# NAIST-Archlab/vsim

Hardware: AMD Instinct MI355X
Metric: decode tokens/sec GPT-J-6B Q4_0 @1 GPU; achieved HBM GB/s vs peak (higher is better)
Workload: dtype f32 (Q4_0 x Q4_0 operands); 1 GPU; gpt-j-6B Q4_0 decode, 874 timed tokens after a 5-token prompt + 5 warm-up tokens, batch 1; mode=exact, n_ctx=980, parallelism=single, graph=True

## Files before the change

vsim_amd/csrc/common.hpp:

```cpp
#pragma once

#include <hip/hip_runtime.h>
#include <stdint.h>

#include <map>
#include <string>

#include "../../include/vsim_hip.h"

namespace vsim {

constexpr int QK = 32;
constexpr int QBYTES = 20;

constexpr int T32 = 32;

typedef float f32x4 __attribute__((ext_vector_type(4)));
typedef unsigned int u32x4 __attribute__((ext_vector_type(4)));

struct W4 {
  const uint8_t *qs;
  const float *d;
  int rows, k, tiles;
  __host__ __device__ int nb() const { return k / QK; }
  __host__ __device__ size_t off(int r, int b) const {
    return ((size_t)(r / T32) * nb() + b) * T32 + (r & (T32 - 1));
  }
};

inline size_t w4_bytes(int rows, int k) { return (size_t)((rows + T32 - 1) / T32) * T32 * (k / QK) * QBYTES; }

inline W4 w4_view(const void *base, int rows, int k) {
  W4 v;
  v.rows = rows;
  v.k = k;
  v.tiles = (rows + T32 - 1) / T32;
  const size_t nblk = (size_t)v.tiles * T32 * (k / QK);
  v.qs = (const uint8_t *)base;
  v.d = (const float *)((const uint8_t *)base + nblk * 16);
  return v;
}

enum { EPI_STORE = 0, EPI_GELU_Q = 1 };
struct GemvJob {
  W4 w;
  const float *xd;
  const uint8_t *xqs;
  const float *xdd;
  const float *bias;
  float *y;
  int epi;
  const uint16_t *gelu_tab;
  uint8_t *oq_qs;
  float *oq_d;
  float *oxd;
};
struct GemvBatch {
  GemvJob j[4];
  int nj;
};

struct LnQuantJob {
  const float *x;
  const float *w, *b;
  uint8_t *qs;
  float *d;
  float *xd;
  const float *ja, *jab, *jf, *jfb;
  float *jout;
  unsigned *ep;
};

struct TailLn {
  const float *x;
  const float *ab, *fb;
  float *jout;
  const float *w1, *b1;
  uint8_t *q1;
  float *d1, *xd1;
  const float *w2, *b2;
  uint8_t *q2;
  float *d2, *xd2;
  unsigned long long *og, *jg;
  uint4 *rec;
  const unsigned *ep;
  unsigned *stats;
  int il;
};
constexpr int LNT_MAX_TILES = 256;

struct AttnJob {
  const float *q, *k, *v;
  float *kc, *vc;
  const int *npast;
  const double2 *cs;
  const uint16_t *etab;
  int d, H, n_rot, style;
  int n_ctx;
  int nsplit;
  int kqv_nth;
  float scale;
  const float *alibi;
  uint8_t *oq_qs;
  float *oq_d, *oxd;
  float *out;
};

constexpr int ATT_VTF = 8192;
__host__ __device__ constexpr int attn_lds_floats(int d, int n_ctx) {
  return ((2 * d + n_ctx + 3) & ~3) + 2 * ATT_VTF;
}

int launch_ln_quant(const LnQuantJob &j0, const LnQuantJob *j1, int n, hipStream_t s);
int launch_residual_join(const float *x, const float *a, const float *ab, const float *f, const float *fb, float *out,
                         int n, hipStream_t s);
int launch_gemv_epi(const GemvBatch &B, int mode, hipStream_t s);
int launch_attn_decode(const AttnJob &A, int n_ctx, hipStream_t s);
struct AttnRows {
  float *const *kc, *const *vc;
  size_t loff;
  const int *npast;
};
int launch_attn_decode_batch(const AttnJob &A, const AttnRows &R, int B, int n_ctx, hipStream_t s);
int launch_gemv_chain_batch(const GemvBatch &B, hipStream_t s);
bool gemv_chain_solo(const GemvBatch &B);

__device__ __forceinline__ float bits_f(uint32_t w) { return __uint_as_float(w); }
__device__ __forceinline__ uint32_t f_bits(float f) { return __float_as_uint(f); }

__device__ __forceinline__ float h2f(uint16_t h) {
  const uint32_t w = (uint32_t)h << 16;
  const uint32_t sign = w & 0x80000000u;
  const uint32_t two_w = w + w;
  const float normalized = bits_f((two_w >> 4) + (0xE0u << 23)) * 0x1.0p-112f;
  const float denormalized = bits_f((two_w >> 17) | (126u << 23)) - 0.5f;
  return bits_f(sign | (two_w < (1u << 27) ? f_bits(denormalized) : f_bits(normalized)));
}

__device__ __forceinline__ uint16_t f2h(float f) {
  float base = (fabsf(f) * 0x1.0p+112f) * 0x1.0p-110f;
  const uint32_t w = f_bits(f);
  const uint32_t shl1_w = w + w;
  const uint32_t sign = w & 0x80000000u;
  uint32_t bias = shl1_w & 0xFF000000u;
  if (bias < 0x71000000u) bias = 0x71000000u;
  base = bits_f((bias >> 1) + 0x07800000u) + base;
  const uint32_t bits = f_bits(base);
  const uint32_t exp_bits = (bits >> 13) & 0x00007C00u;
  const uint32_t mantissa_bits = bits & 0x00000FFFu;
  const uint32_t nonsign = exp_bits + mantissa_bits;
  return (uint16_t)((sign >> 16) | (shl1_w > 0xFF000000u ? 0x7E00u : nonsign));
}

// ... 188 lines not shown
```

vsim_amd/csrc/gemv_chain.hip:

```cpp
#include <cstdlib>
#include <cstring>

#ifdef VSIM_NB_STAMPS
namespace vsim {
__device__ unsigned long long g_nb_stamps[2048][32];
}
#define ATT_STAMP(i) \
  if (threadIdx.x == 0) g_nb_stamps[1536 + blockIdx.x][4 + (i)] = __builtin_amdgcn_s_memrealtime()
#endif
#include "attn.hpp"
#include "kern.hpp"
#include "../../include/vsim_hip.h"

namespace vsim {

typedef const __attribute__((address_space(4))) float sfloat;
typedef const __attribute__((address_space(1))) u32x4 gu32x4;
typedef const __attribute__((address_space(1))) float gfloat;

__device__ __forceinline__ void producer_barrier() { asm volatile("s_barrier" ::: "memory"); }


constexpr int waitcnt_vm(int n) { return 0x0F70 | (n & 15) | ((n >> 4) << 14); }
constexpr int c2_waves(int npw, bool fill) {
// ... 726 lines not shown
        break;
      }
    }
  }
  __syncthreads();
  NBS(if (threadIdx.x == 0) tl[1] = __builtin_amdgcn_s_memrealtime();)
  if (T.lnon)
    chain32_nb_body<C2Tail, true, true, 2>(T.o, b, L.n, T.err, &T.ln);
  else
    chain32_nb_body<C2Tail, true, true>(T.o, b, L.n, T.err);
  NBS(if (threadIdx.x == 0) tl[2] = __builtin_amdgcn_s_memrealtime();)
}

bool tail_ln_ok(int E) {
  int dev = 0, cus = 0;
  if (hipGetDevice(&dev) != hipSuccess || hipDeviceGetAttribute(&cus, hipDeviceAttributeMultiprocessorCount, dev) != hipSuccess)
    return false;
  return E % T32 == 0 && E / T32 <= LNT_MAX_TILES && E / T32 < cus;
}

int launch_layer_tail(const GemvBatch &f, const GemvBatch &o, const AttnJob &a, const TailSync &sy, int n_ctx,
                      hipStream_t s, const TailLn *ln) {
  const int S = a.nsplit > 1 ? a.nsplit : 1;
  if (a.d % 32 != 0 || a.d > 256 || a.n_ctx != n_ctx || a.d % S != 0 || (a.d / S) % QK != 0 ||
      (size_t)attn_lds_floats(a.d, n_ctx) * sizeof(float) > sizeof(NbLds<C2Tail>)) {
    set_error("layer tail: attention shape (head dim, n_ctx) outside the fused kernel's range");
    return VSIM_EINVAL;
  }
  if (f.nj > 1 || o.nj > 1) {
    set_error("layer tail: fc_out and the out-projection are one job each");
    return VSIM_EINVAL;
  }
  TailJob T{};
  T.f = f;
  T.o = o;
  T.a = a;
  T.sy = sy;
  if (!sy.hflag || !sy.ep || sy.il < 0 || sy.il > 254 || a.H * S > TAIL_MAX_HEADS) {
    set_error("layer tail: the heads' flags need a flag buffer, the step epoch, a layer below 255, at most 128 heads");
    return VSIM_EINVAL;
  }
  T.err = spin_error_counter();
  T.nf = 0;
  if (ln) {
    const int E = o.nj == 1 ? o.j[0].w.rows : 0;
    if (f.nj != 1 || o.nj != 1 || f.j[0].w.rows != E || a.d * a.H != E || !tail_ln_ok(E) || ln->il < 0 ||
        ln->il > 254 || !ln->x || !ln->jout || !ln->w1 || !ln->b1 || !ln->q1 || !ln->d1 || !ln->xd1 || !ln->og ||
        !ln->jg || !ln->rec || !ln->ep || (ln->w2 && (!ln->b2 || !ln->q2 || !ln->d2 || !ln->xd2))) {
      set_error("layer tail: the in-tail LayerNorm needs fc_out and the out-projection over E rows, E/32 below the CU count");
      return VSIM_EINVAL;
    }
    T.lnon = 1;
    T.ln = *ln;
  }
  for (int i = 0; i < f.nj; ++i) T.nf += f.j[i].w.tiles;
  int no = 0;
  for (int i = 0; i < o.nj; ++i) no += o.j[i].w.tiles;
  const dim3 grid(T.nf + a.H * S + no), blk(C2Tail::THREADS);
  constexpr size_t pad = sizeof(NbLds<C2Tail>) > 80 * 1024 ? 0 : 81 * 1024 - sizeof(NbLds<C2Tail>);
  hipLaunchKernelGGL(k_layer_tail, grid, blk, pad, s, T);
  VSIM_HIP(hipGetLastError());
  return VSIM_OK;
}

template <int CB, int CONS = 1>
struct SoloShape {
  static constexpr int CP = CB * 16, LD = CP + 4;
  static constexpr int PRODUCERS = CB * CONS;
  static constexpr int WAVES = PRODUCERS + (PRODUCERS + 2) / 3;
  static constexpr int ROWS = 64 * CONS;
  static constexpr int WIN = 12;
  static_assert(CP / 4 % WIN == 0, "the read window must tile the chunk");
  static_assert(WAVES <= 16, "workgroup size");
  static_assert((WAVES + 3) / 4 >= CONS, "consumer waves on one SIMD");
};
constexpr int C5_RING = 3;

template <int CB, int PF, int CONS>
__device__ __forceinline__ void solo_body(const GemvBatch &B, int g, float (*P)[SoloShape<CB, CONS>::ROWS * SoloShape<CB, CONS>::LD]) {
  using S = SoloShape<CB, CONS>;
  constexpr int TPG = 2 * CONS;
  const int wave = __builtin_amdgcn_readfirstlane(threadIdx.x >> 6);
  const int lane = threadIdx.x & 63;
  int ji = 0;
  while (ji < B.nj) {
    const int ng = (B.j[ji].w.tiles + TPG - 1) / TPG;
    if (g < ng) break;
    g -= ng;
    ++ji;
  }
  if (ji >= B.nj) return;
  ji = __builtin_amdgcn_readfirstlane(ji);
  g = __builtin_amdgcn_readfirstlane(g);
  const int tiles = B.j[ji].w.tiles, nb = B.j[ji].w.k / QK, nch = (nb + CB - 1) / CB;
  const int nit = (nch + 2 + PF) / (PF + 1) * (PF + 1);
  NBS(if (lane == 0 && gridDim.x < 512 && wave < 32) g_nb_stamps[512 + blockIdx.x][wave] =
          (unsigned long long)__builtin_amdgcn_s_getreg(0xF804) | (unsigned long long)__builtin_amdgcn_s_getreg(0xF814) << 32;)

  if ((wave & 3) == 0 && (wave >> 2) >= CONS) {
    for (int k = 0; k < nit; ++k) __syncthreads();
    return;
  }
  if ((wave & 3) != 0) {
    const int pi = wave - 1 - (wave >> 2);
    const int o = pi % CB, c = pi / CB;
    const int h = lane >> 5, r = lane & 31;
    const int tile = TPG * g + 2 * c + h;
    const bool tile_ok = tile < tiles;
    const int tl = tile_ok ? tile : tiles - 1;
    const uint8_t *qs = B.j[ji].w.qs + ((size_t)tl * nb * T32 + r) * 16;
    const float *dd = B.j[ji].w.d + (size_t)tl * nb * T32 + r;
    const float *xg = B.j[ji].xd;
    auto ld = [&](int c, u32x4 &qv, float &dv) {
      const int b = min(c * CB + o, nb - 1);
      qv = __builtin_nontemporal_load((gu32x4 *)(qs + (size_t)b * (T32 * 16)));
      dv = __builtin_nontemporal_load((gfloat *)(dd + (size_t)b * T32));
    };
    auto ldx = [&](int c, f32x2 *xv) {
      const int b = min(c * CB + o, nb - 1);
      const sfloat *xp = (const sfloat *)(xg + (size_t)b * QK);
#pragma unroll
      for (int i = 0; i < 16; ++i) {
        xv[i].x = xp[2 * i];
        xv[i].y = xp[2 * i + 1];
      }
    };
    int ps = 0;
    NBS(unsigned long long st_fw = 0, st_comp = 0, st_bar = 0, pa = 0, pb = 0, pc = 0, pd = 0;
        auto cyc = []() { return __builtin_amdgcn_s_memtime(); };)
    auto step = [&](int k, const f32x2 *xc, f32x2 *xn, const u32x4 &qc, float dqc, u32x4 &qn, float &dqn) {
      ld(k + PF, qn, dqn);
      NBS(const unsigned long long c0 = cyc();)
      __builtin_amdgcn_s_waitcnt(0xC07F);
      NBS(if (pa) { st_fw += pb - pa; st_comp += pc - pb; st_bar += pd - pc; }
          pa = c0; pb = cyc();)
      __builtin_amdgcn_sched_barrier(0);
      ldx(k + 1, xn);
      __builtin_amdgcn_sched_barrier(0);
      {
        const float dv = tile_ok && k * CB + o < nb ? dqc : 0.0f;
        const float dl = 512.0f * dv, ml = -8.0f * dv;
        float dh, mh;
        asm("v_mov_b32 %0, %1" : "=v"(dh) : "v"(dl));
        asm("v_mov_b32 %0, %1" : "=v"(mh) : "v"(ml));
        const f32x2 d2 = {dl, dh}, m2 = {ml, mh};
        float *dst = &P[ps][(64 * c + lane) * S::LD + o * 16];
#pragma unroll
        for (int wv = 0; wv < 4; ++wv) {
          float p4[4];
          pair_terms4_x(qc[wv], d2, m2, xc + 4 * wv, p4);
          *(float4 *)(dst + 4 * wv) = make_float4(p4[0], p4[1], p4[2], p4[3]);
        }
      }
      ps = ps == C5_RING - 1 ? 0 : ps + 1;
      __builtin_amdgcn_sched_barrier(0);
      NBS(pc = cyc();)
      producer_barrier();
      NBS(pd = cyc();)
    };
    u32x4 q[PF + 1];
    float e[PF + 1];
#pragma unroll
    for (int c = 0; c < PF; ++c) ld(c, q[c], e[c]);
    f32x2 xa[16], xb[16];
    ldx(0, xa);
#pragma unroll
    for (int i = 0; i < 16; ++i) asm volatile("" ::"s"(xa[i].x), "s"(xa[i].y));
    static_assert((PF + 1) % 2 == 0, "two factor sets alternate");
    for (int k = 0; k < nit; k += PF + 1) {
#pragma unroll
      for (int u = 0; u < PF + 1; u += 2) {
        step(k + u, xa, xb, q[u], e[u], q[(u + PF) % (PF + 1)], e[(u + PF) % (PF + 1)]);
        step(k + u + 1, xb, xa, q[u + 1], e[u + 1], q[u % (PF + 1)], e[u % (PF + 1)]);
      }
    }
    NBS(if (lane == 0 && gridDim.x < 512 && pi < 6) {
      unsigned long long *st = g_nb_stamps[512 + blockIdx.x] + 12 + 3 * pi;
      st[0] = st_fw;
      st[1] = st_comp;
      st[2] = st_bar;
    })
    return;
  }

  float acc = 0.0f;
  float4 win[S::WIN];
  NBS(unsigned long long sc_bar = 0;
      auto ccyc = []() { return __builtin_amdgcn_s_memtime(); };)
  const int crow = 64 * wave / 4 + lane;
  auto src = [&](int c) { return &P[c % C5_RING][crow * S::LD]; };
  __builtin_amdgcn_s_setprio(3);
  NBS(const unsigned long long c_m0 = __builtin_amdgcn_s_memtime(), c_r0 = __builtin_amdgcn_s_memrealtime();)
  for (int k = 0; k < nit; ++k) {
    const int c = k - 2;
    if (c == -1 && nch > 0) {
      const float *p0 = src(0);
#pragma unroll
      for (int j = 0; j < S::WIN; ++j) win[j] = *(const float4 *)(p0 + 4 * j);
    } else if (c >= 0 && c < nch) {
      const float *pc = src(c), *pn = src(c + 1);
#pragma unroll
      for (int j0 = 0; j0 < S::CP / 4; j0 += 6) {
#pragma unroll
        for (int j = j0; j < j0 + 6; ++j) {
          const float4 v = win[j % S::WIN];
          acc = acc + v.x;
          acc = acc + v.y;
          acc = acc + v.z;
          acc = acc + v.w;
        }
#pragma unroll
        for (int j = j0; j < j0 + 6; ++j) {
          const int jn = j + S::WIN;
          win[j % S::WIN] = jn < S::CP / 4 ? *(const float4 *)(pc + 4 * jn) : *(const float4 *)(pn + 4 * (jn - S::CP / 4));
        }
        __builtin_amdgcn_sched_group_barrier(0x002, 24, 0);
        __builtin_amdgcn_sched_group_barrier(0x100, 6, 0);
      }
    }
    NBS(const unsigned long long b0 = ccyc();)
    __syncthreads();
    NBS(sc_bar += ccyc() - b0;)
  }
  NBS(if (lane == 0 && wave == 0 && gridDim.x < 512) {
    g_nb_stamps[512 + blockIdx.x][30] = sc_bar;
    g_nb_stamps[512 + blockIdx.x][31] = nit;
  })
  NBS(if (lane == 0 && wave == 0 && gridDim.x < 512) {
    unsigned long long *st = g_nb_stamps[512 + blockIdx.x];
    st[8] = c_m0;
    st[9] = __builtin_amdgcn_s_memtime();
    st[10] = c_r0;
    st[11] = __builtin_amdgcn_s_memrealtime();
  })

  const int row = g * S::ROWS + crow;
  const int rows = B.j[ji].w.rows;
  const float *bias = B.j[ji].bias;
  float *y = B.j[ji].y;
  if (B.j[ji].epi == EPI_GELU_Q) {
    const bool ok = row < rows;
    float gv = 0.0f;
    if (ok) {
      gv = h2f(B.j[ji].gelu_tab[f2h(acc + bias[row])]);
      if (y) y[row] = gv;
    }
    const int blk = row / QK;
    quantize_half(gv, lane, ok, B.j[ji].oq_qs + (size_t)blk * 16, B.j[ji].oq_d + blk,
                  B.j[ji].oxd + (size_t)blk * QK);
  } else if (row < rows) {
    y[row] = bias ? acc + bias[row] : acc;
  }
  __builtin_amdgcn_s_setprio(0);
}

template <int CB, int PF, int CONS>
__global__ void __launch_bounds__((64 * SoloShape<CB, CONS>::WAVES), 1) k_gemv_solo(GemvBatch B) {
  __shared__ __attribute__((aligned(16))) float P[C5_RING][SoloShape<CB, CONS>::ROWS * SoloShape<CB, CONS>::LD];
  solo_body<CB, PF, CONS>(B, blockIdx.x, P);
}

static int solo_groups(const GemvBatch &B, int cons = 1) {
  int g = 0;
  for (int i = 0; i < B.nj; ++i) g += (B.j[i].w.tiles + 2 * cons - 1) / (2 * cons);
  return g;
}

constexpr int SOLO_CB = 6, SOLO_PF = 3, SOLO_MIN_GROUPS = 192;

bool gemv_chain_solo(const GemvBatch &B) { return solo_groups(B) >= SOLO_MIN_GROUPS; }

int launch_gemv_chain_batch(const GemvBatch &B, hipStream_t s) {
  int tiles = 0;
  for (int i = 0; i < B.nj; ++i) {
    if (B.j[i].w.k % QK != 0 || B.j[i].w.k <= 0) {
      set_error("gemv: K must be a positive multiple of 32");
      return VSIM_EINVAL;
    }
    if (!B.j[i].xd) { set_error("gemv: exact mode needs the activation factors xd"); return VSIM_EINVAL; }
    tiles += B.j[i].w.tiles;
  }
  if (tiles == 0) return VSIM_OK;
  if (gemv_chain_solo(B)) {
    hipLaunchKernelGGL((k_gemv_solo<SOLO_CB, SOLO_PF, 1>), dim3(solo_groups(B)), dim3(64 * SoloShape<SOLO_CB, 1>::WAVES),
                       0, s, B);
  } else {
    hipLaunchKernelGGL(k_gemv_chain32, dim3(tiles), dim3(C2Gemv::THREADS), 0, s, B);
  }
  VSIM_HIP(hipGetLastError());
  return VSIM_OK;
}

}

#ifdef VSIM_NB_STAMPS
extern "C" int vsim_debug_nb_stamps(void *dst, size_t bytes) {
  if (bytes > sizeof(vsim::g_nb_stamps)) bytes = sizeof(vsim::g_nb_stamps);
  return hipMemcpyFromSymbol(dst, HIP_SYMBOL(vsim::g_nb_stamps), bytes) == hipSuccess ? 0 : -2;
}
#endif
```

vsim_amd/csrc/kern.hpp:

```cpp
#pragma once

#include <type_traits>

#include "common.hpp"

namespace vsim {

__host__ __device__ constexpr int xd_slot(int l) { return (l & ~3) | ((l & 1) << 1) | ((l >> 1) & 1); }

__device__ __forceinline__ float q4_block(const float *v, uint32_t w[4], float *out) {
  float amax = 0.0f;
#pragma unroll
  for (int l = 0; l < QK; ++l) amax = amax > fabsf(v[l]) ? amax : fabsf(v[l]);
  const float d = amax / 7.0f;
  const float id = d != 0.0f ? 1.0f / d : 0.0f;
#pragma unroll
  for (int i = 0; i < 4; ++i) w[i] = 0;
#pragma unroll
  for (int l = 0; l < QK; l += 2) {
    const int q0 = x86_round_i8(v[l] * id) + 8;
    const int q1 = x86_round_i8(v[l + 1] * id) + 8;
    w[l / 8] |= (uint32_t)((q0 & 0xF) | ((q1 & 0xF) << 4)) << (8 * ((l / 2) & 3));
    out[l] = d * (float)(q0 - 8);
    out[l + 1] = d * (float)(q1 - 8);
  }
  return d;
}

__device__ __forceinline__ void quantize_block(const float *v, uint8_t *qs_out, float *d_out, float *xd_out) {
  uint32_t w[4];
  float out[QK];
  const float d = q4_block(v, w, out);
  *(uint4 *)qs_out = make_uint4(w[0], w[1], w[2], w[3]);
  *d_out = d;
  if (xd_out) {
    float4 *o = (float4 *)xd_out;
#pragma unroll
    for (int i = 0; i < QK / 4; ++i) o[i] = make_float4(out[4 * i], out[4 * i + 2], out[4 * i + 1], out[4 * i + 3]);
  }
}

__device__ __forceinline__ unsigned long long am_key(float v, int i) {
  uint32_t u = __float_as_uint(v);
  if (v != v) u = 0xFFFFFFFFu;
  else if (v == 0.0f) u = 0x80000000u;
  else u = (u & 0x80000000u) ? ~u : (u | 0x80000000u);
  return ((unsigned long long)u << 32) | (0xFFFFFFFFu - (uint32_t)i);
}

__device__ __forceinline__ void pair_terms4(uint32_t w, float d0, const float *x8, float *p4) {
  const uint32_t lo = w & 0x0F0F0F0Fu, hi = (w >> 4) & 0x0F0F0F0Fu;
#pragma unroll
  for (int k = 0; k < 4; ++k) {
    const float n0 = __uint_as_float(__builtin_amdgcn_perm(0x4B4B4B4Bu, lo, 0x040C0C00u | k)) - 8388616.0f;
    const float n1 = __uint_as_float(__builtin_amdgcn_perm(0x4B4B4B4Bu, hi, 0x040C0C00u | k)) - 8388616.0f;
    const float f0 = d0 * n0, f1 = d0 * n1;
    p4[k] = f0 * x8[2 * k] + f1 * x8[2 * k + 1];
  }
}

typedef float f32x2 __attribute__((ext_vector_type(2)));

template <int K>
__device__ __forceinline__ float cvt_ubyte(uint32_t w) {
  float f;
  if (K == 0) asm("v_cvt_f32_ubyte0 %0, %1" : "=v"(f) : "v"(w));
  if (K == 1) asm("v_cvt_f32_ubyte1 %0, %1" : "=v"(f) : "v"(w));
  if (K == 2) asm("v_cvt_f32_ubyte2 %0, %1" : "=v"(f) : "v"(w));
  if (K == 3) asm("v_cvt_f32_ubyte3 %0, %1" : "=v"(f) : "v"(w));
  return f;
}

__device__ __forceinline__ void pair_terms4_fma(uint32_t w, f32x2 d2, f32x2 m2, const f32x2 *x4, float *p4) {
  const uint32_t lo = w & 0x0F0F0F0Fu, hi = (w >> 4) & 0x0F0F0F0Fu;
  auto term = [&](auto kc) {
    constexpr int k = decltype(kc)::value;
    f32x2 n;
    n.x = cvt_ubyte<k>(lo);
    n.y = cvt_ubyte<k>(hi);
    const f32x2 f = __builtin_elementwise_fma(n, d2, m2);
    const f32x2 t = f * x4[k];
    p4[k] = t.x + t.y;
  };
  term(std::integral_constant<int, 0>{});
  term(std::integral_constant<int, 1>{});
  term(std::integral_constant<int, 2>{});
  term(std::integral_constant<int, 3>{});
}

__device__ __forceinline__ void pair_terms4_x(uint32_t w, f32x2 d512, f32x2 m2, const f32x2 *xw, float *p4) {
  const int lo = (int)(w & 0x0F0F0F0Fu), hi = (int)((w >> 4) & 0x0F0F0F0Fu);
  const f32x2 f01 = __builtin_elementwise_fma(__builtin_amdgcn_cvt_pk_f32_fp8(lo, false), d512, m2);
  const f32x2 g01 = __builtin_elementwise_fma(__builtin_amdgcn_cvt_pk_f32_fp8(hi, false), d512, m2);
  const f32x2 f23 = __builtin_elementwise_fma(__builtin_amdgcn_cvt_pk_f32_fp8(lo, true), d512, m2);
  const f32x2 g23 = __builtin_elementwise_fma(__builtin_amdgcn_cvt_pk_f32_fp8(hi, true), d512, m2);
  const f32x2 t01 = f01 * xw[0] + g01 * xw[1];
  const f32x2 t23 = f23 * xw[2] + g23 * xw[3];
  p4[0] = t01.x;
  p4[1] = t01.y;
  p4[2] = t23.x;
  p4[3] = t23.y;
}

template <int POS>
__device__ __forceinline__ float xbcast(float f0, float f1) {
  return __int_as_float(__builtin_amdgcn_update_dpp(0, __float_as_int(POS < 16 ? f0 : f1), 0x150 + (POS & 15), 0xF, 0xF,
                                                    false));
}
template <int W>
__device__ __forceinline__ void pair_terms4_dpp(uint32_t w, f32x2 d512, f32x2 m2, float F0, float F1, float *p4) {
  const int lo = (int)(w & 0x0F0F0F0Fu), hi = (int)((w >> 4) & 0x0F0F0F0Fu);
  const f32x2 f01 = __builtin_elementwise_fma(__builtin_amdgcn_cvt_pk_f32_fp8(lo, false), d512, m2);
  const f32x2 g01 = __builtin_elementwise_fma(__builtin_amdgcn_cvt_pk_f32_fp8(hi, false), d512, m2);
  const f32x2 f23 = __builtin_elementwise_fma(__builtin_amdgcn_cvt_pk_f32_fp8(lo, true), d512, m2);
  const f32x2 g23 = __builtin_elementwise_fma(__builtin_amdgcn_cvt_pk_f32_fp8(hi, true), d512, m2);
  p4[0] = xbcast<xd_slot(8 * W + 0)>(F0, F1) * f01.x + xbcast<xd_slot(8 * W + 1)>(F0, F1) * g01.x;
  p4[1] = xbcast<xd_slot(8 * W + 2)>(F0, F1) * f01.y + xbcast<xd_slot(8 * W + 3)>(F0, F1) * g01.y;
  p4[2] = xbcast<xd_slot(8 * W + 4)>(F0, F1) * f23.x + xbcast<xd_slot(8 * W + 5)>(F0, F1) * g23.x;
  p4[3] = xbcast<xd_slot(8 * W + 6)>(F0, F1) * f23.y + xbcast<xd_slot(8 * W + 7)>(F0, F1) * g23.y;
}

__device__ __forceinline__ uint32_t lds_addr(const void *p) { return (uint32_t)(uintptr_t)p; }

template <bool NT = true>
__device__ __forceinline__ void glds16(const void *g, uint32_t lds) {
  unsigned keep;
  if constexpr (NT)
    asm volatile("s_mov_b32 %0, m0\n\ts_mov_b32 m0, %2\n\ts_nop 0\n\tglobal_load_lds_dwordx4 %1, off nt\n\ts_mov_b32 m0, %0"
                 : "=&s"(keep) : "v"(g), "s"(lds) : "memory");
  else
// ... 33 lines not shown
}

namespace vsim {

__device__ __forceinline__ double rl_d(double v, int l) {
  const long long b = __double_as_longlong(v);
  const int lo = __builtin_amdgcn_readlane((int)(b & 0xFFFFFFFF), l), hi = __builtin_amdgcn_readlane((int)(b >> 32), l);
  return __longlong_as_double(((long long)hi << 32) | (unsigned)lo);
}

__device__ __forceinline__ double seq_sum_exact_inl(const float *row, int n, int lane) {
  constexpr int CAP = 32;
  const int n4 = n / 4;
  double s = 0.0;
  for (int c4 = 0; c4 < n4; c4 += 64) {
    const int i4 = c4 + lane;
    const float4 v = i4 < n4 ? ((const float4 *)row)[i4] : make_float4(0.f, 0.f, 0.f, 0.f);
    const float e[4] = {v.x, v.y, v.z, v.w};
    int um = 1 << 30;
    double sa = 0.0;
#pragma unroll
    for (int k = 0; k < 4; ++k) {
      um = min(um, ulp_exp(e[k]));
      sa += (double)fabsf(e[k]);
    }
    um = wave_min_i(um);
    sa = wave_sum_d(sa);
    const int cn = min(256, n - 4 * c4);
    int b = 0;
    if (um == (1 << 30) || sa * (1.0 + 0x1.0p-30) < ldexp(1.0, 53 + um)) {
      double p[4];
      p[0] = e[0];
#pragma unroll
      for (int k = 1; k < 4; ++k) p[k] = p[k - 1] + (double)e[k];
      double x = p[3];
#pragma unroll
      for (int d = 1; d < 64; d <<= 1) {
        const double t = __shfl_up(x, d, 64);
        if (lane >= d) x += t;
      }
      const double ex = x - p[3];
#pragma unroll
      for (int k = 0; k < 4; ++k) p[k] += ex;
      double pb = 0.0;
      for (int r = 0; r <= CAP; ++r) {
        int jl = 1 << 30;
#pragma unroll
        for (int k = 3; k >= 0; --k) {
          const int j = 4 * lane + k + 1;
          if (j > b && j <= cn) {
            const double d = p[k] - pb, t = s + d, bb = t - s, er = (s - (t - bb)) + (d - bb);
            if (er != 0.0 || t != t) jl = j;
          }
        }
        const int j = wave_min_i(jl);
        if (j == (1 << 30)) {
          s = s + (rl_d(p[3], (cn - 1) >> 2) - pb);
          b = cn;
          break;
        }
        const int kj = (j - 1) & 3;
        const double pj = rl_d(kj == 0 ? p[0] : kj == 1 ? p[1] : kj == 2 ? p[2] : p[3], (j - 1) >> 2);
        s = s + (pj - pb);
        pb = pj;
        b = j;
      }
    }
    if (b < cn) {
      double m = s;
      if (lane == 0)
        for (int j = b; j < cn; ++j) m += (double)row[4 * c4 + j];
      s = rl_d(m, 0);
    }
  }
  return s;
}
__device__ __noinline__ double seq_sum_exact(const float *row, int n, int lane) { return seq_sum_exact_inl(row, n, lane); }

template <int NT, bool CERT = true, int UP = 4>
__device__ void ln_exact_lds_t(const float *__restrict__ x, float *row, int n, const float *__restrict__ gw,
                               const float *__restrict__ gb, unsigned *stats, const float *__restrict__ ja = nullptr,
                               const float *__restrict__ jab = nullptr, const float *__restrict__ jf = nullptr,
                               const float *__restrict__ jfb = nullptr, float *__restrict__ jout = nullptr,
                               int s0 = 0, int s1 = 1 << 30) {
  constexpr int NW = NT / 64;
  __shared__ double shs[NW], shsa[NW];
  __shared__ int shu[NW];
  __shared__ double bcast_d;
  __shared__ float bcast_f;
  const int lane = threadIdx.x & 63, wid = threadIdx.x >> 6;
  const int n4 = n / 4;
  const double eps = 1e-5f;
  double s = 0.0, sa = 0.0;
  int um = 1 << 30;
  const int i0 = max(s0, 0) + (int)threadIdx.x;
  float4 w0 = make_float4(0.f, 0.f, 0.f, 0.f), b0 = w0;
  if (gw && i0 < min(s1, n4)) {
    w0 = ((const float4 *)gw)[i0];
    b0 = ((const float4 *)gb)[i0];
  }
  auto join = [&](int i, float4 v, float4 a, float4 ab, float4 f, float4 fb) {
    if (ja || jf) {
      if (jab) a = make_float4(a.x + ab.x, a.y + ab.y, a.z + ab.z, a.w + ab.w);
      if (jfb) f = make_float4(f.x + fb.x, f.y + fb.y, f.z + fb.z, f.w + fb.w);
      const float4 t = !jf ? a : !ja ? f : make_float4(a.x + f.x, a.y + f.y, a.z + f.z, a.w + f.w);
      v = make_float4(v.x + t.x, v.y + t.y, v.z + t.z, v.w + t.w);
      if (jout && i >= s0 && i < s1) ((float4 *)jout)[i] = v;
    }
    ((float4 *)row)[i] = v;
    const float e[4] = {v.x, v.y, v.z, v.w};
#pragma unroll
    for (int j = 0; j < 4; ++j) {
      s += (double)e[j];
      sa += (double)fabsf(e[j]);
      um = min(um, ulp_exp(e[j]));
    }
  };
  auto ld4 = [](const float *p, int i) {
    return p ? ((const float4 *)p)[i] : make_float4(0.f, 0.f, 0.f, 0.f);
  };
  if (n4 <= UP * NT) {
    float4 v[UP], a[UP], ab[UP], f[UP], fb[UP];
#pragma unroll
    for (int u = 0; u < UP; ++u) {
      const int i = (int)threadIdx.x + u * NT;
      if (i < n4) {
        v[u] = ((const float4 *)x)[i];
        a[u] = ld4(ja, i);
        ab[u] = ld4(jab, i);
        f[u] = ld4(jf, i);
        fb[u] = ld4(jfb, i);
      }
    }
#pragma unroll
    for (int u = 0; u < UP; ++u) {
      const int i = (int)threadIdx.x + u * NT;
      if (i < n4) join(i, v[u], a[u], ab[u], f[u], fb[u]);
    }
  } else {
    for (int i = threadIdx.x; i < n4; i += NT)
      join(i, ((const float4 *)x)[i], ld4(ja, i), ld4(jab, i), ld4(jf, i), ld4(jfb, i));
  }
  s = wave_sum_d(s);
  sa = wave_sum_d(sa);
  um = wave_min_i(um);
  if (lane == 0) {
    shs[wid] = s;
    shsa[wid] = sa;
    shu[wid] = um;
  }
  __syncthreads();
  s = 0.0;
  sa = 0.0;
  um = 1 << 30;
#pragma unroll
  for (int w = 0; w < NW; ++w) {
    s += shs[w];
    sa += shsa[w];
    um = min(um, shu[w]);
  }
  const bool exact = !CERT || (um == (1 << 30)) || sa * (1.0 + 0x1.0p-30) < ldexp(1.0, 53 + um);
  if (!exact) {
    if (wid == 0) {
      const double m = seq_sum_exact(row, n, lane);
      if (lane == 0) {
        bcast_d = m;
        if (stats) atomicAdd(&stats[0], 1u);
      }
    }
    __syncthreads();
    s = bcast_d;
  }
  const double mean = s / n;
  double s2 = 0.0;
  for (int i = threadIdx.x; i < n4; i += NT) {
    const float4 v4 = ((const float4 *)row)[i];
    const float e[4] = {v4.x, v4.y, v4.z, v4.w};
#pragma unroll
    for (int j = 0; j < 4; ++j) {
      const double v = (double)e[j] - mean;
      s2 += v * v;
    }
  }
  s2 = wave_sum_d(s2);
  __syncthreads();
  if (lane == 0) shs[wid] = s2;
  __syncthreads();
  s2 = 0.0;
#pragma unroll
  for (int w = 0; w < NW; ++w) s2 += shs[w];
  const double B = (2.0 * n + 64.0) * 0x1.0p-53 * s2;
  const float sc_lo = (float)(1.0 / sqrt((s2 + B) / n + eps));
  const float sc_hi = (float)(1.0 / sqrt((s2 - B > 0.0 ? s2 - B : 0.0) / n + eps));
  float scale = sc_lo;
  if (CERT && sc_lo != sc_hi) {
    if (threadIdx.x == 0) {
      double q = 0.0;
      for (int i = 0; i < n; ++i) {
        const double v = (double)row[i] - mean;
        q += v * v;
      }
      bcast_f = (float)(1.0 / sqrt(q / n + eps));
      if (stats) atomicAdd(&stats[1], 1u);
    }
    __syncthreads();
    scale = bcast_f;
  }
  for (int i = max(s0, 0) + (int)threadIdx.x; i < min(s1, n4); i += NT) {
    const float4 v4 = ((const float4 *)row)[i];
    float e[4] = {v4.x, v4.y, v4.z, v4.w};
    float4 w4 = w0, b4 = b0;
    if (gw && i != i0) {
      w4 = ((const float4 *)gw)[i];
      b4 = ((const float4 *)gb)[i];
    }
    const float wv[4] = {w4.x, w4.y, w4.z, w4.w}, bv[4] = {b4.x, b4.y, b4.z, b4.w};
#pragma unroll
    for (int j = 0; j < 4; ++j) {
      float v = (float)((double)e[j] - mean);
      v = v * scale;
      if (gw) v = (wv[j] * v) + bv[j];
      e[j] = v;
    }
    ((float4 *)row)[i] = make_float4(e[0], e[1], e[2], e[3]);
  }
  __syncthreads();
}

__device__ __forceinline__ void ln_exact_lds(const float *__restrict__ x, float *row, int n, const float *__restrict__ gw,
                                             const float *__restrict__ gb, unsigned *stats) {
  ln_exact_lds_t<NORM_THREADS>(x, row, n, gw, gb, stats);
}

template <bool CO, typename T>
__device__ __forceinline__ void st_out(T *p, T v) {
  if constexpr (CO) __hip_atomic_store(p, v, __ATOMIC_RELAXED, __HIP_MEMORY_SCOPE_AGENT);
  else *p = v;
}

__device__ __forceinline__ int q4_half(float v, float &d) {
  auto mx = [](float a, float b) { return a > b ? a : b; };
  float a = fabsf(v);
  a = mx(a, dpp::mov<dpp::QP_XOR1, 0xF>(a, 0.0f));
  a = mx(a, dpp::mov<dpp::QP_XOR2, 0xF>(a, 0.0f));
  a = mx(a, dpp::mov<dpp::HALF_MIRROR, 0xF>(a, 0.0f));
  a = mx(a, dpp::mov<dpp::MIRROR, 0xF>(a, 0.0f));
  a = mx(a, __int_as_float(__builtin_amdgcn_ds_swizzle(__float_as_int(a), 0x401F)));
  d = a / 7.0f;
  const float id = d != 0.0f ? 1.0f / d : 0.0f;
  return x86_round_i8(v * id) + 8;
}

template <bool CO = false>
__device__ __forceinline__ void quantize_half(float v, int lane, bool ok, uint8_t *qs_out, float *d_out,
                                              float *xd_out) {
  float d;
  const int q = q4_half(v, d);
  const int l = lane & 31;
  const int qn = dpp::mov<dpp::QP_XOR1, 0xF>(q, 0);
  const uint32_t byte = (l & 1) ? (uint32_t)((qn & 0xF) | ((q & 0xF) << 4)) : (uint32_t)((q & 0xF) | ((qn & 0xF) << 4));
  uint32_t word = byte << (8 * ((l >> 1) & 3));
  word |= (uint32_t)dpp::mov<dpp::QP_XOR2, 0xF>((int)word, 0);
  word |= (uint32_t)dpp::mov<dpp::HALF_MIRROR, 0xF>((int)word, 0);
  if (ok) {
    if ((l & 7) == 0) st_out<CO>((uint32_t *)qs_out + (l >> 3), word);
    if (l == 0) st_out<CO>(d_out, d);
    st_out<CO>(xd_out + xd_slot(l), d * (float)(q - 8));
  }
}

__device__ __forceinline__ void quantize_block_lanes(float v, int lane, uint8_t *qs_out, float *d_out,
                                                     float *xd_out) {
  float a = lane < 32 ? fabsf(v) : 0.0f;
#pragma unroll
  for (int o = 16; o > 0; o >>= 1) {
    const float t = __shfl_xor(a, o, 64);
    a = a > t ? a : t;
  }
  const float amax = a;
  const float d = amax / 7.0f;
  const float id = d != 0.0f ? 1.0f / d : 0.0f;
  const int q = x86_round_i8(v * id) + 8;
  const int qn = __shfl_xor(q, 1, 64);
  const uint32_t byte = (lane & 1) ? 0u : (uint32_t)((q & 0xF) | ((qn & 0xF) << 4));
  uint32_t word = byte << (8 * ((lane >> 1) & 3));
  word |= __shfl_xor(word, 2, 64);
  word |= __shfl_xor(word, 4, 64);
  if (lane < 32) {
    if ((lane & 7) == 0) ((uint32_t *)qs_out)[lane >> 3] = word;
    if (lane == 0) *d_out = d;
    xd_out[xd_slot(lane)] = d * (float)(q - 8);
  }
}

template <int NT>
__device__ __forceinline__ void ln_quant_job(const LnQuantJob &J, float *row, int n, unsigned *stats, int b0, int b1) {
  const int lane = threadIdx.x & 63;
  ln_exact_lds_t<NT>(J.x, row, n, J.w, J.b, stats, J.ja, J.jab, J.jf, J.jfb, J.jout, b0 * QK / 4, b1 * QK / 4);
  for (int b2 = threadIdx.x >> 6; b0 + 2 * b2 < b1; b2 += NT / 64) {
    const int b = b0 + 2 * b2 + (lane >> 5);
    const bool ok = b < b1;
    const float v = ok ? row[b * QK + (lane & 31)] : 0.0f;
    quantize_half(v, lane, ok, J.qs + (size_t)b * 16, J.d + b, J.xd + (size_t)b * QK);
  }
}

}
```

vsim_amd/csrc/model.cpp:

```cpp
#include <hip/hip_runtime.h>

#include <algorithm>
#include <atomic>
#include <cmath>
#include <cstdio>
#include <cstring>
#include <fstream>
#include <map>
#include <string>
#include <vector>

#include "common.hpp"
#include "fast.hpp"
#include "sampler.hpp"
#include "../../include/vsim_hip.h"

using namespace vsim;

namespace {

enum Kind { KQ4 = 0, KF32 = 1 };

struct Slot {
  void *ptr;
// ... 750 lines not shown
    P.xq[0] = q1;
    P.xd[0] = d1;
    P.xq[1] = G.two_norms ? m->xq2 : q1;
    P.xd[1] = G.two_norms ? d2 : d1;
    P.nj = 4;
    P.j[0] = FastJob{w4_view(L.wfc, F, E), L.bfc, nullptr, FE_GELU_Q, 1};
    P.j[1] = FastJob{w4_view(L.wq, E, E), G.qkvo_bias ? L.bq : nullptr, m->Qb, FE_ROPE_Q, 0};
    P.j[2] = FastJob{w4_view(L.wk, E, E), G.qkvo_bias ? L.bk : nullptr, m->kcache + loff, FE_ROPE_K, 0};
    P.j[3] = FastJob{w4_view(L.wv, E, E), G.qkvo_bias ? L.bv : nullptr, m->vcache + loff, FE_V, 0};
    P.gelu_tab = tab.gelu_f16;
    P.clear = m->tail_done;
    P.nclear = 4 * H;
    P.oq_qs = q3;
    P.oq_d = d3;
    P.npast = m->npast_dev;
    P.cs = m->rope_cs;
    P.d = d;
    P.n_rot = m->hp.n_rot;
    P.style = G.rotary == ROT_GPTJ ? 1 : 0;
    LAUNCH(m, nk, launch_fast_gemv(P, E, s), "k_fast_gemv (fc_in, Q, K, V)",
           w4_algo_bytes(P.j[0].w) + 3 * w4_algo_bytes(P.j[1].w));
    FastTail T{};
    T.wf = w4_view(L.wproj, E, F);
    T.xf_qs = q3;
    T.xf_d = d3;
    T.ffp = m->fast_ffp;
    T.sf = fast_sf(m);
    T.q = m->Qb;
    T.kc = m->kcache + loff;
    T.vc = m->vcache + loff;
    T.npast = m->npast_dev;
    T.d = d;
    T.H = H;
    T.nchunk = nchunk;
    T.scale = scale;
    T.part = m->fast_part;
    T.hcnt = m->tail_done;
    T.oq_qs = m->xqa;
    T.oq_d = q4_scales(m->xqa, E);
    FastOproj O{};
    O.w = w4_view(L.wo, E, E);
    O.xq = T.oq_qs;
    O.xd = T.oq_d;
    O.d = d;
    O.bo = G.qkvo_bias ? L.bo : nullptr;
    O.ffp = m->fast_ffp;
    O.sf = fast_sf(m);
    O.bproj = L.bproj;
    O.x = R[cur];
    O.out = R[cur ^ 1];
    LAUNCH(m, nk, launch_fast_tail(T, s), "k_fast_tail (fc_out + attention)", w4_algo_bytes(T.wf) + kv_bytes);
    LAUNCH(m, nk, launch_fast_oproj_join(O, s), "k_fast_oproj_join", w4_algo_bytes(O.w));
    cur ^= 1;
  }
  if (m->last) {
    FastGemv P{};
    P.lnx = R[cur];
    P.lnw[0] = P.lnw[1] = m->lnf_w;
    P.lnb[0] = P.lnb[1] = m->lnf_b;
    P.xq[0] = P.xq[1] = q1;
    P.xd[0] = P.xd[1] = d1;
    P.nj = 1;
    P.j[0] = FastJob{w4_view(m->lmh, V, E), G.lmh_bias ? m->lmh_b : nullptr, m->logits, FE_STORE, 0};
    LAUNCH(m, nk, launch_fast_gemv(P, E, s), "k_fast_gemv (lm_head)", w4_algo_bytes(P.j[0].w));
  }
  m->resid_final = R[cur];
  return VSIM_OK;
}

int enqueue_decode(vsim_model *m, int &nk) {
  if (m->mode == VSIM_MODE_FAST && fast_decode_ok(m)) return enqueue_decode_fast(m, nk);
  const int E = m->hp.n_embd, H = m->hp.n_head, d = E / H, F = 4 * E, V = m->hp.n_vocab;
  const GraphDesc &G = m->gd;
  const bool serial = G.residual != RES_PARALLEL;
  hipStream_t s = m->stream;
  DevTables tab;
  RC(tables_get(&tab));
  uint8_t *q1 = m->xq1, *q2 = m->xq2, *q3 = m->xq3, *qa = m->xqa;
  float *d1 = q4_scales(q1, E), *d2 = q4_scales(q2, E), *d3 = q4_scales(q3, F), *da = q4_scales(qa, E);
  if (m->first && G.emb_norm) {
    RC(launch_get_rows(m->wte, E, V, m->tok_dev, 1, m->cur1, s));
    RC(launch_norm(m->cur1, m->inpL, E, 1, m->emb_w, m->emb_b, s));
    nk += 2;
  } else if (m->first) {
    RC(launch_get_rows(m->wte, E, V, m->tok_dev, 1, m->inpL, s));
    ++nk;
  }
  const float scale = (float)(1.0f / std::sqrt((double)(float(E) / H)));
  const double kv_bytes = 2.0 * ((double)m->prof_npast + 1) * E * sizeof(float);
  auto ln_bytes = [&](int nnorm, bool join) {
    return 4.0 * E * (1 + (join ? 5 : 0) + 3 * nnorm) + 0.625 * E * nnorm;
  };
  float *R[2] = {m->inpL, m->inpL2};
  int cur = 0;
  bool pending = false, ln_done = false;
  const float *pend_a = nullptr, *pend_ab = nullptr, *pend_fb = nullptr;
  auto join_into = [&](LnQuantJob &j, bool write) {
    j.ja = pend_a;
    j.jab = pend_ab;
    j.jf = m->ff;
    j.jfb = pend_fb;
    j.jout = write ? R[cur ^ 1] : nullptr;
  };
  auto job = [&](GemvBatch &Bt, int i, void *W, int M, int K, const float *xd, const uint8_t *xq, const float *xdd,
                 const float *bias, float *y) {
    GemvJob &J = Bt.j[i];
    J.w = w4_view(W, M, K);
    J.xd = xd;
    J.xqs = xq;
    J.xdd = xdd;
    J.bias = bias;
    J.y = y;
    J.epi = EPI_STORE;
  };
  const bool tail = m->mode == VSIM_MODE_EXACT && (size_t)attn_lds_floats(d, m->n_ctx) * sizeof(float) <= 75264;
  const bool lnt_ok = tail && !serial && m->l1 <= 255 && tail_ln_ok(E);
  auto attn_job = [&](size_t loff) {
    AttnJob A{};
    A.q = m->Qb;
    A.k = m->Kb;
    A.v = m->Vb;
    A.kc = m->kcache + loff;
    A.vc = m->vcache + loff;
    A.npast = m->npast_dev;
    A.cs = m->rope_cs;
    A.etab = tab.exp_f16;
    A.d = d;
    A.H = H;
    A.n_rot = G.rotary == ROT_NONE ? 0 : m->hp.n_rot;
    A.style = G.rotary == ROT_GPTJ ? 1 : 0;
    A.n_ctx = m->n_ctx;
    constexpr int ATT_SPLIT = 2;
    A.nsplit = 1;
    for (int sp = tail && !serial ? ATT_SPLIT : 1; sp > 1; --sp)
      if (d % sp == 0 && (d / sp) % QK == 0) {
        A.nsplit = sp;
        break;
      }
    A.scale = m->attn_scale != 0.0f ? m->attn_scale : scale;
    A.kqv_nth = m->kqv_nth;
    A.alibi = G.alibi ? m->alibi : nullptr;
    A.oq_qs = qa;
    A.oq_d = da;
    A.oxd = m->xda;
    A.out = nullptr;
    return A;
  };
  auto gemv = [&](const GemvBatch &Bt, const char *what, double bytes) -> int {
    LAUNCH(m, nk, launch_gemv_epi(Bt, m->mode, s),
           std::string(m->mode != VSIM_MODE_EXACT ? "k_gemv_fast_epi" : gemv_chain_solo(Bt) ? "k_gemv_solo"
                                                                                       : "k_gemv_chain32") +
               " (" + what + ")",
           bytes);
    return VSIM_OK;
  };
  for (int il = m->l0; il < m->l1; ++il) {
    const LayerW &L = m->layers[il - m->l0];
    const size_t loff = (size_t)(il - m->l0) * m->n_ctx * E;
    if (serial) {
      LnQuantJob j1{R[cur], L.ln1_w, L.ln1_b, q1, d1, m->xd1};
      if (pending) join_into(j1, true);
      if (tail && il == m->l0) j1.ep = m->lnt_ep;
      LAUNCH(m, nk, launch_ln_quant(j1, nullptr, E, s), "k_ln_quant", ln_bytes(1, pending));
      if (pending) cur ^= 1;
      GemvBatch B{};
      B.nj = 3;
      job(B, 0, L.wq, E, E, m->xd1, q1, d1, L.bq, m->Qb);
      job(B, 1, L.wk, E, E, m->xd1, q1, d1, L.bk, m->Kb);
      job(B, 2, L.wv, E, E, m->xd1, q1, d1, L.bv, m->Vb);
      RC(gemv(B, "Q, K, V", 3 * w4_algo_bytes(B.j[0].w)));
      const AttnJob A = attn_job(loff);
      GemvBatch Bo{};
      Bo.nj = 1;
      job(Bo, 0, L.wo, E, E, m->xda, qa, da, nullptr, m->attn);
      if (tail) {
        GemvBatch none{};
        LAUNCH(m, nk, launch_layer_tail(none, Bo, A, TailSync{m->tail_hflag, m->lnt_ep, il}, m->n_ctx, s),
               "k_layer_tail (attention + out-proj)", w4_algo_bytes(Bo.j[0].w) + kv_bytes);
      } else {
        LAUNCH(m, nk, launch_attn_decode(A, m->n_ctx, s), "k_attn_decode", kv_bytes);
        RC(gemv(Bo, "out-proj", w4_algo_bytes(Bo.j[0].w)));
      }
      LnQuantJob j2{R[cur], L.ln2_w, L.ln2_b, q2, d2, m->xd2};
      j2.ja = m->attn;
      j2.jab = L.bo;
      j2.jout = G.residual == RES_SERIAL_JOINED ? R[cur ^ 1] : nullptr;
      LAUNCH(m, nk, launch_ln_quant(j2, nullptr, E, s), "k_ln_quant", ln_bytes(1, true));
      if (G.residual == RES_SERIAL_JOINED) cur ^= 1;
      GemvBatch Bi{};
      Bi.nj = 1;
      job(Bi, 0, L.wfc, F, E, m->xd2, q2, d2, L.bfc, nullptr);
      Bi.j[0].epi = EPI_GELU_Q;
      Bi.j[0].gelu_tab = tab.gelu_f16;
      Bi.j[0].oq_qs = q3;
      Bi.j[0].oq_d = d3;
      Bi.j[0].oxd = m->xd3;
      RC(gemv(Bi, "fc_in", w4_algo_bytes(Bi.j[0].w)));
      GemvBatch Bf{};
      Bf.nj = 1;
      job(Bf, 0, L.wproj, E, F, m->xd3, q3, d3, nullptr, m->ff);
      RC(gemv(Bf, "fc_out", w4_algo_bytes(Bf.j[0].w)));
      pending = true;
      pend_a = nullptr;
      pend_ab = nullptr;
      pend_fb = L.bproj;
      continue;
    }
    const TailSync sy{m->tail_hflag, m->lnt_ep, il};
    if (!ln_done) {
      LnQuantJob j1{R[cur], L.ln1_w, L.ln1_b, q1, d1, m->xd1};
      LnQuantJob j2{R[cur], L.ln2_w, L.ln2_b, q2, d2, m->xd2};
      if (pending) {
        join_into(j1, true);
        join_into(j2, false);
      }
      if (tail && il == m->l0) j1.ep = m->lnt_ep;
      LAUNCH(m, nk, launch_ln_quant(j1, G.two_norms ? &j2 : nullptr, E, s), "k_ln_quant",
             ln_bytes(G.two_norms ? 2 : 1, pending));
      if (pending) cur ^= 1;
    }
    ln_done = false;
    GemvBatch B{};
    B.nj = 4;
    job(B, 0, L.wfc, F, E, G.two_norms ? m->xd2 : m->xd1, G.two_norms ? q2 : q1, G.two_norms ? d2 : d1, L.bfc, nullptr);
    B.j[0].epi = EPI_GELU_Q;
    B.j[0].gelu_tab = tab.gelu_f16;
    B.j[0].oq_qs = q3;
    B.j[0].oq_d = d3;
    B.j[0].oxd = m->xd3;
    job(B, 1, L.wq, E, E, m->xd1, q1, d1, G.qkvo_bias ? L.bq : nullptr, m->Qb);
    job(B, 2, L.wk, E, E, m->xd1, q1, d1, G.qkvo_bias ? L.bk : nullptr, m->Kb);
    job(B, 3, L.wv, E, E, m->xd1, q1, d1, G.qkvo_bias ? L.bv : nullptr, m->Vb);
    LAUNCH(m, nk, launch_gemv_epi(B, m->mode, s),
           m->mode == VSIM_MODE_EXACT ? "k_gemv_solo (fc_in, Q, K, V)" : "k_gemv_fast_epi (fc_in, Q, K, V)",
           w4_algo_bytes(B.j[0].w) + 3 * w4_algo_bytes(B.j[1].w));
    const AttnJob A = attn_job(loff);
    GemvBatch Bf{}, Bo{};
    Bf.nj = 1;
    job(Bf, 0, L.wproj, E, F, m->xd3, q3, d3, nullptr, m->ff);
    Bo.nj = 1;
    job(Bo, 0, L.wo, E, E, m->xda, qa, da, nullptr, m->attn);
    const bool lnt = tail && lnt_ok && (il + 1 < m->l1 || m->last);
    if (lnt) {
      TailLn N{};
      N.x = R[cur];
      N.ab = G.qkvo_bias ? L.bo : nullptr;
      N.fb = L.bproj;
      N.jout = R[cur ^ 1];
      if (il + 1 < m->l1) {
        const LayerW &Ln = m->layers[il + 1 - m->l0];
        N.w1 = Ln.ln1_w;
        N.b1 = Ln.ln1_b;
        if (G.two_norms) {
          N.w2 = Ln.ln2_w;
          N.b2 = Ln.ln2_b;
          N.q2 = q2;
          N.d2 = d2;
          N.xd2 = m->xd2;
        }
      } else {
        N.w1 = m->lnf_w;
        N.b1 = m->lnf_b;
      }
      N.q1 = q1;
      N.d1 = d1;
      N.xd1 = m->xd1;
      N.og = m->lnt_og;
      N.jg = m->lnt_jg;
      N.rec = m->lnt_rec;
      N.ep = m->lnt_ep;
      N.stats = dev_stats();
      N.il = il;
      LAUNCH(m, nk, launch_layer_tail(Bf, Bo, A, sy, m->n_ctx, s, &N),
             "k_layer_tail (fc_out + attention + out-proj + join + LayerNorm)",
             w4_algo_bytes(Bf.j[0].w) + w4_algo_bytes(Bo.j[0].w) + kv_bytes + ln_bytes(N.w2 ? 2 : 1, true));
      cur ^= 1;
      ln_done = true;
      pending = false;
      continue;
    }
    if (tail) {
      LAUNCH(m, nk, launch_layer_tail(Bf, Bo, A, sy, m->n_ctx, s), "k_layer_tail (fc_out + attention + out-proj)",
             w4_algo_bytes(Bf.j[0].w) + w4_algo_bytes(Bo.j[0].w) + kv_bytes);
    } else {
      LAUNCH(m, nk, launch_attn_decode(A, m->n_ctx, s), "k_attn_decode", kv_bytes);
      Bf.j[1] = Bo.j[0];
      Bf.nj = 2;
      LAUNCH(m, nk, launch_gemv_epi(Bf, m->mode, s),
             m->mode == VSIM_MODE_EXACT ? "k_gemv_chain32 (fc_out, out-proj)" : "k_gemv_fast_epi (fc_out, out-proj)",
             w4_algo_bytes(Bf.j[0].w) + w4_algo_bytes(Bf.j[1].w));
    }
    pending = true;
    pend_a = m->attn;
    pend_ab = G.qkvo_bias ? L.bo : nullptr;
    pend_fb = L.bproj;
  }
  if (m->last) {
// ... 1115 lines not shown
```

Before: 547.1 tokens/s.

## Fuse token embedding lookup into first layernorm and hoist solo GEMV job lookup

Removes the separate get_rows launch for the first layer by having the first ln_quant kernel dequantize the token's embedding row directly from the Q4 table and write it to the residual buffer. Separately, the solo GEMV kernel now picks its job with a branchless prefix-sum instead of a loop, pins job parameters in scalar registers, and loads the bias before the main loop so it is not fetched after the reduction. The cost is one fewer kernel per token plus a shorter epilogue, in exchange for more scalar register pressure and a more complex layernorm input path.

```diff
diff --git a/vsim_amd/csrc/common.hpp b/vsim_amd/csrc/common.hpp
--- a/vsim_amd/csrc/common.hpp
+++ b/vsim_amd/csrc/common.hpp
@@ -69,6 +69,8 @@
   const float *ja, *jab, *jf, *jfb;
   float *jout;
   unsigned *ep;
+  W4 emb;
+  const int32_t *tok;
 };
 
 struct TailLn {
diff --git a/vsim_amd/csrc/gemv_chain.hip b/vsim_amd/csrc/gemv_chain.hip
--- a/vsim_amd/csrc/gemv_chain.hip
+++ b/vsim_amd/csrc/gemv_chain.hip
@@ -832,16 +832,18 @@
   constexpr int TPG = 2 * CONS;
   const int wave = __builtin_amdgcn_readfirstlane(threadIdx.x >> 6);
   const int lane = threadIdx.x & 63;
-  int ji = 0;
-  while (ji < B.nj) {
-    const int ng = (B.j[ji].w.tiles + TPG - 1) / TPG;
-    if (g < ng) break;
-    g -= ng;
-    ++ji;
-  }
-  if (ji >= B.nj) return;
+  const int nj = B.nj, t0 = B.j[0].w.tiles, t1 = B.j[1].w.tiles, t2 = B.j[2].w.tiles, t3 = B.j[3].w.tiles;
+  asm volatile("" ::"s"(nj), "s"(t0), "s"(t1), "s"(t2), "s"(t3));
+  const int e1 = (t0 + TPG - 1) / TPG;
+  const int e2 = e1 + (nj > 1 ? (t1 + TPG - 1) / TPG : 0);
+  const int e3 = e2 + (nj > 2 ? (t2 + TPG - 1) / TPG : 0);
+  const int e4 = e3 + (nj > 3 ? (t3 + TPG - 1) / TPG : 0);
+  if (nj < 1 || g >= e4) return;
+  int ji = g < e1 ? 0 : g < e2 ? 1 : g < e3 ? 2 : 3;
+  g -= ji == 0 ? 0 : ji == 1 ? e1 : ji == 2 ? e2 : e3;
   ji = __builtin_amdgcn_readfirstlane(ji);
   g = __builtin_amdgcn_readfirstlane(g);
+  asm volatile("" ::"s"(B.j[ji].w.qs), "s"(B.j[ji].w.d), "s"(B.j[ji].w.k), "s"(B.j[ji].w.tiles), "s"(B.j[ji].xd));
   const int tiles = B.j[ji].w.tiles, nb = B.j[ji].w.k / QK, nch = (nb + CB - 1) / CB;
   const int nit = (nch + 2 + PF) / (PF + 1) * (PF + 1);
   NBS(if (lane == 0 && gridDim.x < 512 && wave < 32) g_nb_stamps[512 + blockIdx.x][wave] =
@@ -939,6 +941,16 @@
       auto ccyc = []() { return __builtin_amdgcn_s_memtime(); };)
   const int crow = 64 * wave / 4 + lane;
   auto src = [&](int c) { return &P[c % C5_RING][crow * S::LD]; };
+  const int row = g * S::ROWS + crow;
+  const int rows = B.j[ji].w.rows, epi = B.j[ji].epi;
+  const float *bias = B.j[ji].bias;
+  float *y = B.j[ji].y;
+  const uint16_t *gelu_tab = B.j[ji].gelu_tab;
+  uint8_t *oq_qs = B.j[ji].oq_qs;
+  float *oq_d = B.j[ji].oq_d, *oxd = B.j[ji].oxd;
+  asm volatile("" ::"s"(rows), "s"(epi), "s"(bias), "s"(y), "s"(gelu_tab), "s"(oq_qs), "s"(oq_d), "s"(oxd));
+  const bool biased = bias && row < rows;
+  const float bv = biased ? bias[row] : 0.0f;
   __builtin_amdgcn_s_setprio(3);
   NBS(const unsigned long long c_m0 = __builtin_amdgcn_s_memtime(), c_r0 = __builtin_amdgcn_s_memrealtime();)
   for (int k = 0; k < nit; ++k) {
@@ -984,22 +996,17 @@
     st[11] = __builtin_amdgcn_s_memrealtime();
   })
 
-  const int row = g * S::ROWS + crow;
-  const int rows = B.j[ji].w.rows;
-  const float *bias = B.j[ji].bias;
-  float *y = B.j[ji].y;
-  if (B.j[ji].epi == EPI_GELU_Q) {
+  if (epi == EPI_GELU_Q) {
     const bool ok = row < rows;
     float gv = 0.0f;
     if (ok) {
-      gv = h2f(B.j[ji].gelu_tab[f2h(acc + bias[row])]);
+      gv = h2f(gelu_tab[f2h(acc + bv)]);
       if (y) y[row] = gv;
     }
     const int blk = row / QK;
-    quantize_half(gv, lane, ok, B.j[ji].oq_qs + (size_t)blk * 16, B.j[ji].oq_d + blk,
-                  B.j[ji].oxd + (size_t)blk * QK);
+    quantize_half(gv, lane, ok, oq_qs + (size_t)blk * 16, oq_d + blk, oxd + (size_t)blk * QK);
   } else if (row < rows) {
-    y[row] = bias ? acc + bias[row] : acc;
+    y[row] = biased ? acc + bv : acc;
   }
   __builtin_amdgcn_s_setprio(0);
 }
diff --git a/vsim_amd/csrc/kern.hpp b/vsim_amd/csrc/kern.hpp
--- a/vsim_amd/csrc/kern.hpp
+++ b/vsim_amd/csrc/kern.hpp
@@ -46,6 +46,18 @@
   else if (v == 0.0f) u = 0x80000000u;
   else u = (u & 0x80000000u) ? ~u : (u | 0x80000000u);
   return ((unsigned long long)u << 32) | (0xFFFFFFFFu - (uint32_t)i);
+}
+
+__device__ __forceinline__ float4 w4_row4(const W4 &W, int r, int i) {
+  if (r < 0 || r >= W.rows) {
+    const float q = __builtin_nanf("");
+    return make_float4(q, q, q, q);
+  }
+  const size_t off = W.off(r, i / (QK / 4));
+  const float d = W.d[off];
+  const uint32_t q = *(const uint16_t *)(W.qs + off * 16 + 2 * (i % (QK / 4)));
+  return make_float4((float)((int)(q & 0xF) - 8) * d, (float)((int)((q >> 4) & 0xF) - 8) * d,
+                     (float)((int)((q >> 8) & 0xF) - 8) * d, (float)((int)(q >> 12) - 8) * d);
 }
 
 __device__ __forceinline__ void pair_terms4(uint32_t w, float d0, const float *x8, float *p4) {
@@ -245,7 +257,9 @@
                                const float *__restrict__ gb, unsigned *stats, const float *__restrict__ ja = nullptr,
                                const float *__restrict__ jab = nullptr, const float *__restrict__ jf = nullptr,
                                const float *__restrict__ jfb = nullptr, float *__restrict__ jout = nullptr,
-                               int s0 = 0, int s1 = 1 << 30) {
+                               int s0 = 0, int s1 = 1 << 30, const W4 *emb = nullptr, const int32_t *tok = nullptr) {
+  const int er = emb ? *tok : 0;
+  auto ldx = [&](int i) { return emb ? w4_row4(*emb, er, i) : ((const float4 *)x)[i]; };
   constexpr int NW = NT / 64;
   __shared__ double shs[NW], shsa[NW];
   __shared__ int shu[NW];
@@ -269,6 +283,8 @@
       const float4 t = !jf ? a : !ja ? f : make_float4(a.x + f.x, a.y + f.y, a.z + f.z, a.w + f.w);
       v = make_float4(v.x + t.x, v.y + t.y, v.z + t.z, v.w + t.w);
       if (jout && i >= s0 && i < s1) ((float4 *)jout)[i] = v;
+    } else if (emb && jout && i >= s0 && i < s1) {
+      ((float4 *)jout)[i] = v;
     }
     ((float4 *)row)[i] = v;
     const float e[4] = {v.x, v.y, v.z, v.w};
@@ -288,7 +304,7 @@
     for (int u = 0; u < UP; ++u) {
       const int i = (int)threadIdx.x + u * NT;
       if (i < n4) {
-        v[u] = ((const float4 *)x)[i];
+        v[u] = ldx(i);
         a[u] = ld4(ja, i);
         ab[u] = ld4(jab, i);
         f[u] = ld4(jf, i);
@@ -302,7 +318,7 @@
     }
   } else {
     for (int i = threadIdx.x; i < n4; i += NT)
-      join(i, ((const float4 *)x)[i], ld4(ja, i), ld4(jab, i), ld4(jf, i), ld4(jfb, i));
+      join(i, ldx(i), ld4(ja, i), ld4(jab, i), ld4(jf, i), ld4(jfb, i));
   }
   s = wave_sum_d(s);
   sa = wave_sum_d(sa);
@@ -459,7 +475,8 @@
 template <int NT>
 __device__ __forceinline__ void ln_quant_job(const LnQuantJob &J, float *row, int n, unsigned *stats, int b0, int b1) {
   const int lane = threadIdx.x & 63;
-  ln_exact_lds_t<NT>(J.x, row, n, J.w, J.b, stats, J.ja, J.jab, J.jf, J.jfb, J.jout, b0 * QK / 4, b1 * QK / 4);
+  ln_exact_lds_t<NT>(J.x, row, n, J.w, J.b, stats, J.ja, J.jab, J.jf, J.jfb, J.jout, b0 * QK / 4, b1 * QK / 4,
+                     J.emb.qs ? &J.emb : nullptr, J.tok);
   for (int b2 = threadIdx.x >> 6; b0 + 2 * b2 < b1; b2 += NT / 64) {
     const int b = b0 + 2 * b2 + (lane >> 5);
     const bool ok = b < b1;
diff --git a/vsim_amd/csrc/model.cpp b/vsim_amd/csrc/model.cpp
--- a/vsim_amd/csrc/model.cpp
+++ b/vsim_amd/csrc/model.cpp
@@ -856,10 +856,13 @@
     RC(launch_get_rows(m->wte, E, V, m->tok_dev, 1, m->cur1, s));
     RC(launch_norm(m->cur1, m->inpL, E, 1, m->emb_w, m->emb_b, s));
     nk += 2;
-  } else if (m->first) {
-    RC(launch_get_rows(m->wte, E, V, m->tok_dev, 1, m->inpL, s));
-    ++nk;
-  }
+  }
+  const bool emb_ln = m->first && !G.emb_norm;
+  auto emb_into = [&](LnQuantJob &j, float *out) {
+    j.emb = w4_view(m->wte, V, E);
+    j.tok = m->tok_dev;
+    j.jout = out;
+  };
   const float scale = (float)(1.0f / std::sqrt((double)(float(E) / H)));
   const double kv_bytes = 2.0 * ((double)m->prof_npast + 1) * E * sizeof(float);
   auto ln_bytes = [&](int nnorm, bool join) {
@@ -934,6 +937,7 @@
     if (serial) {
       LnQuantJob j1{R[cur], L.ln1_w, L.ln1_b, q1, d1, m->xd1};
       if (pending) join_into(j1, true);
+      if (emb_ln && il == m->l0) emb_into(j1, R[cur]);
       if (tail && il == m->l0) j1.ep = m->lnt_ep;
       LAUNCH(m, nk, launch_ln_quant(j1, nullptr, E, s), "k_ln_quant", ln_bytes(1, pending));
       if (pending) cur ^= 1;
@@ -987,6 +991,10 @@
       if (pending) {
         join_into(j1, true);
         join_into(j2, false);
+      }
+      if (emb_ln && il == m->l0) {
+        emb_into(j1, R[cur]);
+        emb_into(j2, nullptr);
       }
       if (tail && il == m->l0) j1.ep = m->lnt_ep;
       LAUNCH(m, nk, launch_ln_quant(j1, G.two_norms ? &j2 : nullptr, E, s), "k_ln_quant",
```

New measurement: 552.5 tokens/s, median of 6. No clear change (+1.0%).
